# Tai-Wang/Depth-from-Motion

Hardware: NVIDIA H100
Metric: frames/sec (higher is better)
Workload: dtype f32 (bf16x2 split operands, fp32 accumulate)

## Files before the change

depth_from_motion_b200/csrc/conv_tc.cuh:

```cuda
#pragma once
#include <cuda.h>
#include <cuda_bf16.h>

#include <algorithm>
#include <cstdlib>
#include <type_traits>
#include <vector>

#include "common.cuh"
#include "simt_kernels.cuh"
#include "wgmma.cuh"

namespace dfm {

inline uint16_t bf16_rn_bits(float f) {
  uint32_t u;
  memcpy(&u, &f, 4);
  if ((u & 0x7F800000u) == 0x7F800000u) return (uint16_t)(u >> 16);
  u += 0x7FFFu + ((u >> 16) & 1u);
  return (uint16_t)(u >> 16);
}
inline float bf16_bits_to_float(uint16_t b) {
  uint32_t u = (uint32_t)b << 16;
  float f;
  memcpy(&f, &u, 4);
  return f;
}

inline int tc_sm_count() {
  int& cached = per_device<int, 1>();
  if (!cached) cudaDeviceGetAttribute(&cached, cudaDevAttrMultiProcessorCount, cur_device());
  return cached;
}

enum { TC_S1 = 0, TC_S2 = 1, TC_T = 2 };
constexpr int TC_BX = 8, TC_BY = 16;
constexpr int TC_MMA_THREADS = 256;
constexpr int TC_LOAD_THREADS = 256;
constexpr int TC_THREADS = TC_MMA_THREADS + TC_LOAD_THREADS;
constexpr int TC_MAXOPS = 9, TC_MAXBLK = 48;
constexpr int TC_ZERO_TAP = 255;

template <int MODE>
struct TcMode;
template <>
struct TcMode<TC_S1> {
  static constexpr int PXB = 10, PYB = 18, PITCH = 10, ROWS = 186, CG = 32, NSTAGE = 4;
  static constexpr int SLOT_BLOCKS = 1;
  __host__ __device__ static int zo_of(int zi, int dz) { return zi + dz; }
  __host__ __device__ static int zi_first(int zo) { return zo - 1; }
  __host__ __device__ static int zi_last(int zo) { return zo + 1; }
  __host__ __device__ static int ptype(int) { return 0; }
};
template <>
struct TcMode<TC_S2> {
  static constexpr int PXB = 17, PYB = 33, PITCH = 9, ROWS = 620, CG = 16, NSTAGE = 3;
  static constexpr int SLOT_BLOCKS = 1;
  __host__ __device__ static int zo_of(int zi, int dz) { return (zi >> 1) + dz; }
  __host__ __device__ static int zi_first(int zo) { return 2 * zo - 1; }
  __host__ __device__ static int zi_last(int zo) { return 2 * zo + 1; }
  __host__ __device__ static int ptype(int zi) { return zi & 1; }
};
template <>
struct TcMode<TC_T> {
  static constexpr int PXB = 9, PYB = 17, PITCH = 9, ROWS = 154, CG = 32, NSTAGE = 4;
  static constexpr int SLOT_BLOCKS = 4;
  __host__ __device__ static int zo_of(int zi, int dz) { return 2 * zi + dz; }
  __host__ __device__ static int zi_first(int zo) { return zo >> 1; }
  __host__ __device__ static int zi_last(int zo) { return (zo + 1) >> 1; }
  __host__ __device__ static int ptype(int) { return 0; }
};

inline int tc_mode_of(const ConvGeom& g) {
  if (g.transposed) return TC_T;
  if (g.sd == 1 && g.sh == 1 && g.sw == 1 && g.pd == 1 && g.ph == 1 && g.pw == 1) return TC_S1;
  if (g.sd == 2 && g.sh == 2 && g.sw == 2 && g.pd == 1 && g.ph == 1 && g.pw == 1 &&
      g.Di % 2 == 0 && g.Hi % 2 == 0 && g.Wi % 2 == 0)
    return TC_S2;
  return -1;
}
inline bool tc_supported(int Cin, int Cout, int ) {
  if (Cin != 32 && Cin != 64) return false;
  const int ncta = 1024 / Cin;
  return Cout % ncta == 0 && Cout <= 64;
}
inline bool tc_geom_supported(const ConvGeom& g) { return tc_mode_of(g) >= 0; }

struct TcOp {
  uint32_t a_off;
  uint32_t b_off;
  uint32_t b_lbo;
  uint16_t blk0, blk1;
  uint32_t nruns;
  uint32_t runs[3];
};
struct TcBlk {
  int8_t dz;
  uint8_t colblk;
  uint8_t tap;
  uint8_t pad;
};
struct TcProgram {
  int nops;
  uint32_t need;
  TcOp ops[TC_MAXOPS];
  TcBlk blks[TC_MAXBLK];
};

template <int MODE>
inline void tc_build_program(int ptype, int Cin, int ncta, uint32_t* w_cursor, TcProgram* pr) {
  using M = TcMode<MODE>;
  pr->nops = 0;
  pr->need = 0;
  int nb = 0;
  auto add_op = [&](int a_rows, std::vector<TcBlk> blks) {
    TcOp& op = pr->ops[pr->nops++];
    op.a_off = (uint32_t)a_rows * 16;
    op.b_off = *w_cursor;
    op.b_lbo = (uint32_t)blks.size() * ncta * 16;
    op.blk0 = (uint16_t)nb;
    for (TcBlk b : blks) pr->blks[nb++] = b;
    op.blk1 = (uint16_t)nb;
    *w_cursor += (uint32_t)(Cin / 8) * op.b_lbo;
    op.nruns = 0;
    size_t i = 0;
    while (i < blks.size()) {
      size_t e = i + 1;
      auto lin = [&](const TcBlk& b) { return (b.dz + 1) * M::SLOT_BLOCKS + b.colblk; };
      while (e < blks.size() && lin(blks[e]) == lin(blks[i]) + (int)(e - i)) ++e;
      const int nblk = (int)(e - i);
      op.runs[op.nruns++] = (uint32_t)nblk | ((uint32_t)i << 4) | ((uint32_t)lin(blks[i]) << 10);
      for (size_t k = i; k < e; ++k) pr->need |= 1u << (blks[k].dz + 1);
      i = e;
    }
  };
  if (MODE == TC_S1) {
    for (int t = 0; t < 9; ++t) {
      const int dy = t / 3, dx = t % 3;
      add_op(dy * M::PITCH + dx, {TcBlk{-1, 0, (uint8_t)(18 + t), 0}, TcBlk{0, 0, (uint8_t)(9 + t), 0},
                                  TcBlk{1, 0, (uint8_t)t, 0}});
    }
  } else if (MODE == TC_S2) {
    for (int t = 0; t < 9; ++t) {
      const int dy = t / 3, dx = t % 3;
      const int a_rows = (((dx & 1) * 2 + (dy & 1)) * 17 + (dy >> 1)) * M::PITCH + (dx >> 1);
      if (ptype == 0)
        add_op(a_rows, {TcBlk{0, 0, (uint8_t)(9 + t), 0}});
      else
        add_op(a_rows, {TcBlk{0, 0, (uint8_t)(18 + t), 0}, TcBlk{1, 0, (uint8_t)t, 0}});
    }
  } else {
    const int cls_px[4] = {0, 1, 1, 0}, cls_py[4] = {0, 0, 1, 1};
    for (int sh = 0; sh < 4; ++sh) {
      const int sx = sh & 1, sy = sh >> 1;
      std::vector<TcBlk> blks;
      for (int dz = -1; dz <= 1; ++dz) {
        const int kz = dz + 1;
        for (int c = 0; c < 4; ++c) {
          const int px = cls_px[c], py = cls_py[c];
          int kx = -1, ky = -1;
          if (px == 0) { if (!sx) kx = 1; } else kx = sx ? 0 : 2;
          if (py == 0) { if (!sy) ky = 1; } else ky = sy ? 0 : 2;
          const bool real = kx >= 0 && ky >= 0;
          blks.push_back(TcBlk{(int8_t)dz, (uint8_t)c,
                               (uint8_t)(real ? kz * 9 + ky * 3 + kx : TC_ZERO_TAP), 0});
        }
      }
      if (sh == 3) {
        std::vector<TcBlk> real;
        for (const TcBlk& b : blks)
          if (b.tap != TC_ZERO_TAP) real.push_back(b);
        blks = real;
      } else {
        while (!blks.empty() && blks.front().tap == TC_ZERO_TAP) blks.erase(blks.begin());
        while (!blks.empty() && blks.back().tap == TC_ZERO_TAP) blks.pop_back();
      }
      add_op(sy * M::PITCH + sx, blks);
    }
  }
}

struct TcWeights {
  uint8_t* dev = nullptr;
  int Cin = 0, Cout = 0, ncta = 0, nsplit = 0, mode = -1, kslice = 0;
  uint32_t image_bytes = 0, hi_bytes = 0;
  TcProgram prog[2];

  bool ready() const { return dev != nullptr; }
  void release() {
    if (dev) cudaFree(dev);
    dev = nullptr;
  }
  template <int MODE>
  bool build_mode(const float* packed, int cin, int cout, std::string* err, bool ks = false) {
    release();
    mode = MODE;
    Cin = cin;
    Cout = cout;
    kslice = ks ? 1 : 0;
    const int cin_img = ks ? 16 : cin;
    ncta = ks ? cout : 1024 / cin;
    nsplit = ks ? cin / 16 : cout / ncta;
    uint32_t cursor = 0;
    const int ntypes = MODE == TC_S2 ? 2 : 1;
    for (int t = 0; t < ntypes; ++t) tc_build_program<MODE>(t, cin_img, ncta, &cursor, &prog[t]);
    hi_bytes = cursor;
    image_bytes = 2 * hi_bytes;
    std::vector<uint16_t> img((size_t)nsplit * image_bytes / 2);
    const int kch = cin_img / 8;
    for (int s = 0; s < nsplit; ++s)
      for (int t = 0; t < ntypes; ++t)
        for (int o = 0; o < prog[t].nops; ++o) {
          const TcOp& op = prog[t].ops[o];
          const int nblk = op.blk1 - op.blk0;
          for (int kc = 0; kc < kch; ++kc)
            for (int b = 0; b < nblk; ++b)
              for (int j = 0; j < ncta; ++j)
                for (int e = 0; e < 8; ++e) {
                  const int tap = prog[t].blks[op.blk0 + b].tap;
                  if (tap == TC_ZERO_TAP) continue;
                  const int ci = kc * 8 + e + (ks ? s * 16 : 0), co = ks ? j : s * ncta + j;
                  const float w = packed[((size_t)tap * cin + ci) * cout + co];
                  const uint16_t hi = bf16_rn_bits(w);
                  const uint16_t lo = bf16_rn_bits(w - bf16_bits_to_float(hi));
                  const size_t off = (size_t)s * image_bytes / 2 + op.b_off / 2 +
                                     ((size_t)kc * nblk * ncta + (size_t)b * ncta + j) * 8 + e;
                  img[off] = hi;
                  img[off + hi_bytes / 2] = lo;
                }
        }
    if (cudaMalloc(&dev, img.size() * 2) != cudaSuccess ||
        cudaMemcpy(dev, img.data(), img.size() * 2, cudaMemcpyHostToDevice) != cudaSuccess) {
      if (err) *err = "TcWeights: device upload failed";
      release();
      return false;
    }
    return true;
  }
  bool build(const float* packed, int cin, int cout, int m, std::string* err) {
    static const bool no_ks1 = getenv("DFM_NO_KSLICE") != nullptr;
    static const bool ks1 = getenv("DFM_KSLICE_S1") != nullptr;
    if (m == TC_S1) return build_mode<TC_S1>(packed, cin, cout, err,
                                             cin == 64 && cout == 64 && !no_ks1 && ks1);
    if (m == TC_S2) {
      static const bool no_ks = getenv("DFM_NO_KSLICE") != nullptr;
      return build_mode<TC_S2>(packed, cin, cout, err, cout == 64 && !no_ks);
    }
    return build_mode<TC_T>(packed, cin, cout, err);
  }
};

__device__ __forceinline__ uint32_t smem_u32(const void* p) {
  return static_cast<uint32_t>(__cvta_generic_to_shared(p));
}
__device__ __forceinline__ void mbar_init(uint32_t bar, uint32_t count) {
  asm volatile("mbarrier.init.shared::cta.b64 [%0], %1;" ::"r"(bar), "r"(count));
}
__device__ __forceinline__ void mbar_arrive(uint32_t bar) {
  asm volatile("mbarrier.arrive.shared::cta.b64 _, [%0];" ::"r"(bar) : "memory");
}
__device__ __forceinline__ void mbar_wait(uint32_t bar, uint32_t parity, int* err) {
  for (int it = 0; it < (1 << 26); ++it) {
    uint32_t ok;
    asm volatile(
        "{\n\t.reg .pred q;\n\t"
        "mbarrier.try_wait.parity.shared::cta.b64 q, [%1], %2;\n\t"
        "selp.u32 %0, 1, 0, q;\n\t}\n"
        : "=r"(ok)
        : "r"(bar), "r"(parity)
        : "memory");
    if (ok) return;
  }
  *reinterpret_cast<volatile int*>(err) = 1;
  __threadfence_system();
}
__device__ __forceinline__ void mbar_wait_timed(uint32_t bar, uint32_t parity, int* err,
                                                unsigned long long& acc, bool timed) {
  if (!timed) {
    mbar_wait(bar, parity, err);
    return;
  }
  const long long t0 = clock64();
  mbar_wait(bar, parity, err);
  acc += (unsigned long long)(clock64() - t0);
}
__device__ __forceinline__ bool elect_one() {
  uint32_t pred;
  asm volatile(
      "{\n\t.reg .pred p;\n\telect.sync _|p, 0xffffffff;\n\tselp.u32 %0, 1, 0, p;\n\t}\n"
      : "=r"(pred));
  return pred != 0;
}
__device__ __forceinline__ void desc_add(uint64_t& d, uint32_t inc16) {
  asm("{\n\t.reg .b32 lo, hi;\n\tmov.b64 {lo, hi}, %0;\n\tadd.u32 lo, lo, %1;\n\t"
      "mov.b64 %0, {lo, hi};\n\t}\n"
      : "+l"(d)
      : "r"(inc16));
}
__device__ __forceinline__ uint64_t pack64(uint32_t lo, uint32_t hi) {
  return ((uint64_t)hi << 32) | lo;
}
__device__ __forceinline__ void split_store(const float v[8], uint8_t* hi_dst, uint8_t* lo_dst) {
  uint32_t h[4], l[4];
#pragma unroll
  for (int i = 0; i < 4; ++i) {
    const __nv_bfloat162 hh = __floats2bfloat162_rn(v[2 * i], v[2 * i + 1]);
    const float2 hf = __bfloat1622float2(hh);
    const __nv_bfloat162 ll = __floats2bfloat162_rn(v[2 * i] - hf.x, v[2 * i + 1] - hf.y);
    h[i] = *reinterpret_cast<const uint32_t*>(&hh);
    l[i] = *reinterpret_cast<const uint32_t*>(&ll);
  }
  *reinterpret_cast<uint4*>(hi_dst) = make_uint4(h[0], h[1], h[2], h[3]);
  *reinterpret_cast<uint4*>(lo_dst) = make_uint4(l[0], l[1], l[2], l[3]);
}

#ifndef DFM_LD_VARIANT
#define DFM_LD_VARIANT 0
#endif
__device__ __forceinline__ float4 ld_act(const float4* p) {
#if DFM_LD_VARIANT == 1
  return __ldcg(p);
#elif DFM_LD_VARIANT == 2
  float4 v;
  asm volatile("ld.global.nc.L1::no_allocate.L2::256B.v4.f32 {%0,%1,%2,%3}, [%4];"
               : "=f"(v.x), "=f"(v.y), "=f"(v.z), "=f"(v.w) : "l"(p));
  return v;
#elif DFM_LD_VARIANT == 3
  return __ldcs(p);
#elif DFM_LD_VARIANT == 4
  float4 v;
  asm volatile("ld.global.nc.L1::no_allocate.v4.f32 {%0,%1,%2,%3}, [%4];"
               : "=f"(v.x), "=f"(v.y), "=f"(v.z), "=f"(v.w) : "l"(p));
  return v;
#else
  return __ldg(p);
#endif
}

template <int NT>
struct SrcLoader8 {
  static constexpr bool kTma = false;
  Src s;
  int C, H, W;
  static constexpr int BATCH = 6 / NT;
  struct Raw {
    float4 a[NT][2];
  };
  __device__ __forceinline__ void issue(int z, int y, int x, int c0, Raw& r) const {
    const long long inpl = ((long long)y * W + x) * C + c0, plane = (long long)H * W * C;
#pragma unroll
    for (int t = 0; t < NT; ++t) {
      const float* px = s.t[t].x + term_plane(s.t[t], z) * plane + inpl;
      r.a[t][0] = ld_act(reinterpret_cast<const float4*>(px));
      r.a[t][1] = ld_act(reinterpret_cast<const float4*>(px) + 1);
    }
  }
  __device__ __forceinline__ void finish(const Raw& r, int c0, float v[8]) const {
#pragma unroll
    for (int i = 0; i < 8; ++i) v[i] = 0.f;
#pragma unroll
    for (int t = 0; t < NT; ++t) {
      {
        float u[8] = {r.a[t][0].x, r.a[t][0].y, r.a[t][0].z, r.a[t][0].w,
                      r.a[t][1].x, r.a[t][1].y, r.a[t][1].z, r.a[t][1].w};
        if (s.t[t].scale) {
          const float4 s0 = __ldg(reinterpret_cast<const float4*>(s.t[t].scale + c0));
          const float4 s1 = __ldg(reinterpret_cast<const float4*>(s.t[t].scale + c0) + 1);
          const float4 h0 = __ldg(reinterpret_cast<const float4*>(s.t[t].shift + c0));
          const float4 h1 = __ldg(reinterpret_cast<const float4*>(s.t[t].shift + c0) + 1);
          const float sc[8] = {s0.x, s0.y, s0.z, s0.w, s1.x, s1.y, s1.z, s1.w};
          const float sh[8] = {h0.x, h0.y, h0.z, h0.w, h1.x, h1.y, h1.z, h1.w};
#pragma unroll
          for (int i = 0; i < 8; ++i) u[i] = fmaf(u[i], sc[i], sh[i]);
        }
        if (s.t[t].relu) {
#pragma unroll
          for (int i = 0; i < 8; ++i) u[i] = fmaxf(u[i], 0.f);
        }
#pragma unroll
        for (int i = 0; i < 8; ++i) v[i] += u[i];
      }
    }
    if (s.outer_relu) {
#pragma unroll
      for (int i = 0; i < 8; ++i) v[i] = fmaxf(v[i], 0.f);
    }
  }
};

struct WarpLoader8 {
  static constexpr bool kTma = false;
  WarpLoader w;
  static constexpr int BATCH = 1;
  struct Raw {
    float4 t[4][2];
    float wt[4];
  };
  __device__ __forceinline__ void issue(int z, int y, int x, int c0, Raw& r) const {
    c0 += w.first;
    if (c0 < w.C) {
      const float* p = w.cur + ((long long)(y * w.g.step) * w.g.Wf + x * w.g.step) * w.C + c0;
      r.t[0][0] = __ldg(reinterpret_cast<const float4*>(p));
      r.t[0][1] = __ldg(reinterpret_cast<const float4*>(p) + 1);
      r.wt[0] = 1.f;
      r.wt[1] = r.wt[2] = r.wt[3] = 0.f;
      return;
    }
    c0 -= w.C;
    float fx, fy;
    warp_coord(w.g, x, y, __ldg(w.depths + z), fx, fy);
    const Taps t = bilinear_taps(fx, fy, w.g.Hf, w.g.Wf);
#pragma unroll
    for (int k = 0; k < 4; ++k) {
      r.wt[k] = t.w[k];
      if (t.w[k] != 0.f) {
        const float* p = w.prev + (long long)t.off[k] * w.C + c0;
        r.t[k][0] = __ldg(reinterpret_cast<const float4*>(p));
        r.t[k][1] = __ldg(reinterpret_cast<const float4*>(p) + 1);
      }
    }
  }
  __device__ __forceinline__ void finish(const Raw& r, int, float v[8]) const {
#pragma unroll
    for (int i = 0; i < 8; ++i) v[i] = 0.f;
#pragma unroll
    for (int k = 0; k < 4; ++k) {
      if (r.wt[k] != 0.f) {
        v[0] = fmaf(r.wt[k], r.t[k][0].x, v[0]); v[1] = fmaf(r.wt[k], r.t[k][0].y, v[1]);
        v[2] = fmaf(r.wt[k], r.t[k][0].z, v[2]); v[3] = fmaf(r.wt[k], r.t[k][0].w, v[3]);
        v[4] = fmaf(r.wt[k], r.t[k][1].x, v[4]); v[5] = fmaf(r.wt[k], r.t[k][1].y, v[5]);
        v[6] = fmaf(r.wt[k], r.t[k][1].z, v[6]); v[7] = fmaf(r.wt[k], r.t[k][1].w, v[7]);
      }
    }
  }
};

struct TmaLoader8 {
  static constexpr bool kTma = true;
  static constexpr int BATCH = 1;
  CUtensorMap map;
  int nch_total;
  struct Raw {};
  __device__ __forceinline__ void issue(int, int, int, int, Raw&) const {}
  __device__ __forceinline__ void finish(const Raw&, int, float v[8]) const {
#pragma unroll
    for (int i = 0; i < 8; ++i) v[i] = 0.f;
  }
};
constexpr int TMA_S2_CLS = 17 * 9;
constexpr int TMA_S2_CLSR = (2 * TMA_S2_CLS + 7) / 8 * 8;

__device__ __forceinline__ void tma_load_4d(uint32_t dst, const CUtensorMap* map, int c1, int c2,
                                            int c3, uint32_t bar) {
  asm volatile(
      "cp.async.bulk.tensor.4d.shared::cluster.global.tile.mbarrier::complete_tx::bytes "
      "[%0], [%1, {%2, %3, %4, %5}], [%6];" ::"r"(dst),
      "l"(map), "r"(0), "r"(c1), "r"(c2), "r"(c3), "r"(bar)
      : "memory");
}

constexpr int PS_XRUN = 64, PS_WARPS = 4, PS_SEG = 33;
inline size_t presplit_smem_bytes(int C) { return (size_t)PS_WARPS * 4 * (C / 8) * PS_SEG * 16; }
template <int NT>
__global__ void __launch_bounds__(32 * PS_WARPS)
presplit_kernel(const SrcLoader8<NT> ld, int Z, uint4* __restrict__ out) {
  extern __shared__ uint4 ps_sm[];
  const int nch = ld.C >> 3, W = ld.W, H = ld.H, W2 = W >> 1, H2 = H >> 1;
  const int warp = threadIdx.x >> 5, lane = threadIdx.x & 31;
  uint4* sm = ps_sm + (size_t)warp * 4 * nch * PS_SEG;
  const int runs_per_row = (W + PS_XRUN - 1) / PS_XRUN;
  const long long nruns = (long long)Z * H * runs_per_row;
  for (long long r = (long long)blockIdx.x * PS_WARPS + warp; r < nruns;
       r += (long long)gridDim.x * PS_WARPS) {
    const int run = (int)(r % runs_per_row);
    const long long zy = r / runs_per_row;
    const int y = (int)(zy % H), z = (int)(zy / H);
    const int xb = run * PS_XRUN;
#pragma unroll 4
    for (int i = lane; i < PS_XRUN * nch; i += 32) {
      const int xl = i / nch, chunk = i - xl * nch, x = xb + xl;
      if (x < W) {
        typename SrcLoader8<NT>::Raw raw;
        ld.issue(z, y, x, chunk * 8, raw);
        float val[8];
        ld.finish(raw, chunk * 8, val);
        uint4* hi = sm + ((xl & 1) * nch + chunk) * PS_SEG + (xl >> 1);
        split_store(val, reinterpret_cast<uint8_t*>(hi),
                    reinterpret_cast<uint8_t*>(hi + 2 * nch * PS_SEG));
      }
    }
    __syncwarp();
    const int py = y & 1, y2 = y >> 1, x2 = (xb >> 1) + lane;
    for (int seg = 0; seg < 4 * nch; ++seg) {
      const int chunk = seg % nch, px = (seg / nch) & 1, hl = seg / (2 * nch);
      if (2 * x2 + px < W)
        out[((((long long)(z * 2 + hl) * 4 + py * 2 + px) * nch + chunk) * H2 + y2) * W2 + x2] =
            sm[seg * PS_SEG + lane];
    }
    __syncwarp();
  }
}
inline bool presplit_launch(const Src& s, int C, int Z, int H, int W, uint4* out, cudaStream_t st) {
  if ((H | W) & 1) return false;
  const size_t smem = presplit_smem_bytes(C);
  const long long nruns = (long long)Z * H * ((W + PS_XRUN - 1) / PS_XRUN);
  const int blocks = (int)std::min<long long>((nruns + PS_WARPS - 1) / PS_WARPS, 12LL * tc_sm_count());
  auto go = [&](auto kern, auto ld) {
    if (cudaFuncSetAttribute(kern, cudaFuncAttributeMaxDynamicSharedMemorySize, (int)smem) !=
        cudaSuccess)
      return false;
    kern<<<blocks, 32 * PS_WARPS, smem, st>>>(ld, Z, out);
    return cudaGetLastError() == cudaSuccess;
  };
  if (s.n == 1) return go(presplit_kernel<1>, SrcLoader8<1>{s, C, H, W});
  if (s.n == 2) return go(presplit_kernel<2>, SrcLoader8<2>{s, C, H, W});
  return go(presplit_kernel<3>, SrcLoader8<3>{s, C, H, W});
}

inline bool make_presplit_map_s2(CUtensorMap* map, const void* base, int W, int H,
                                 long long slabs, std::string* err) {
  typedef CUresult (*EncodeFn)(CUtensorMap*, CUtensorMapDataType, cuuint32_t, void*,
                               const cuuint64_t*, const cuuint64_t*, const cuuint32_t*,
                               const cuuint32_t*, CUtensorMapInterleave, CUtensorMapSwizzle,
                               CUtensorMapL2promotion, CUtensorMapFloatOOBfill);
  static EncodeFn encode = nullptr;
  if (!encode) {
    void* fn = nullptr;
    cudaDriverEntryPointQueryResult qres;
    if (cudaGetDriverEntryPoint("cuTensorMapEncodeTiled", &fn, cudaEnableDefault, &qres) !=
            cudaSuccess || !fn || qres != cudaDriverEntryPointSuccess) {
      if (err) *err = "cuTensorMapEncodeTiled is not available from this driver";
      return false;
    }
    encode = (EncodeFn)fn;
  }
  const int W2 = W / 2, H2 = H / 2;
  const cuuint64_t dims[4] = {8, (cuuint64_t)W2, (cuuint64_t)H2, (cuuint64_t)slabs};
  const cuuint64_t strides[3] = {16, (cuuint64_t)W2 * 16, (cuuint64_t)H2 * W2 * 16};
  const cuuint32_t box[4] = {8, 9, 17, 2};
  const cuuint32_t estr[4] = {1, 1, 1, 1};
  const CUresult r = encode(map, CU_TENSOR_MAP_DATA_TYPE_UINT16, 4, const_cast<void*>(base), dims,
                            strides, box, estr, CU_TENSOR_MAP_INTERLEAVE_NONE,
                            CU_TENSOR_MAP_SWIZZLE_NONE, CU_TENSOR_MAP_L2_PROMOTION_L2_128B,
                            CU_TENSOR_MAP_FLOAT_OOB_FILL_NONE);
  if (r != CUDA_SUCCESS) {
    if (err) *err = "cuTensorMapEncodeTiled failed with code " + std::to_string((int)r);
    return false;
  }
  return true;
}

struct TcParams {
  const uint8_t* wimg;
  float* out;
  double* stats;
  int Di, Hi, Wi;
  int Do, Ho, Wo, Cout;
  int Mx, My;
  int tiles_x, tiles_y, nsplit;
  int z_unit;
  uint32_t w_bytes, w_hi_bytes;
  int* err;
  unsigned long long* role_cycles;
  const float* addend;
  int zw_lo, zw_hi;
  float zw;
  long long slice_stride;
  int store1;
  int dbg;
};

struct TcItem {
  int x0, y0, split, z_lo, z_hi;
};
struct TcWalk {
  long long cur, end;
  int split;
};
__device__ __forceinline__ TcWalk tc_walk_begin(const TcParams& p) {
  TcWalk w;
  const int per_split = gridDim.x / p.nsplit;
  w.split = blockIdx.x % p.nsplit;
  const int r = blockIdx.x / p.nsplit;
  const long long units_col = p.Do / p.z_unit;
  const long long total = (long long)p.tiles_x * p.tiles_y * units_col;
  w.cur = total * r / per_split;
  w.end = total * (r + 1) / per_split;
  return w;
}
__device__ __forceinline__ bool tc_walk_next(const TcParams& p, TcWalk& w, TcItem& it) {
  if (w.cur >= w.end) return false;
  const long long units_col = p.Do / p.z_unit;
  const int col = (int)(w.cur / units_col);
  const long long u0 = w.cur % units_col;
  const long long u1 = min(units_col, u0 + (w.end - w.cur));
  it.split = w.split;
  it.x0 = (col % p.tiles_x) * TC_BX;
  it.y0 = (col / p.tiles_x) * TC_BY;
  it.z_lo = (int)u0 * p.z_unit;
  it.z_hi = (int)u1 * p.z_unit;
  w.cur += u1 - u0;
  return true;
}

template <int MODE>
struct TcWin;
template <>
struct TcWin<TC_S1> {
  static constexpr int NPL = 3;
  __device__ static int base(int zi) { return zi - 1; }
};
template <>
struct TcWin<TC_S2> {
  static constexpr int NPL = 2;
  __device__ static int base(int zi) { return zi >> 1; }
};
template <>
struct TcWin<TC_T> {
  static constexpr int NPL = 3;
  __device__ static int base(int zi) { return 2 * zi - 1; }
};

template <int MODE, int CIN, int NCTA, class Loader>
__global__ void __launch_bounds__(TC_THREADS, 1) conv_tc_kernel(const __grid_constant__ TcParams p,
                                                                 const __grid_constant__ Loader ld) {
  using M = TcMode<MODE>;
  using Win = TcWin<MODE>;
  constexpr bool TMA = Loader::kTma;
  static_assert(!TMA || MODE == TC_S2, "the TMA loader serves the stride-2 brick only");
  constexpr int CG = M::CG < CIN ? M::CG : CIN;
  constexpr int NCH = CG / 8;
  constexpr int NCG = CIN / CG;
  static_assert(!TMA || NCH == 2, "TMA stride-2 stages hold two 8-channel chunks");
  constexpr uint32_t S2_CLS16 = TMA ? TMA_S2_CLSR : TMA_S2_CLS;
  constexpr uint32_t A_LBO = TMA ? TMA_S2_CLS * 16 : M::ROWS * 16;
  constexpr uint32_t A_SBO = M::PITCH * 16;
  constexpr uint32_t A_HL = TMA ? 4 * TMA_S2_CLSR * 16 : NCH * M::ROWS * 16;
  constexpr uint32_t STAGE_BYTES = 2 * A_HL;
  constexpr uint32_t B_SBO = 128;
  constexpr bool KSLICE = CIN == 16;
  constexpr int NPOS = M::PXB * M::PYB;
  constexpr int LGROUPS = 2;
  constexpr int LG_THREADS = TC_LOAD_THREADS / LGROUPS;
  constexpr int NITEM = (NPOS * NCH + LG_THREADS - 1) / LG_THREADS;
  constexpr int PCOLS = M::SLOT_BLOCKS * NCTA;
  constexpr int NACC = Win::NPL * PCOLS / 2;

  extern __shared__ __align__(1024) uint8_t smem[];
  uint8_t* w_s = smem;
  uint8_t* a_s = smem + p.w_bytes;
  uint64_t* bars = reinterpret_cast<uint64_t*>(a_s + M::NSTAGE * STAGE_BYTES);

  const int tid = threadIdx.x, lane = tid & 31;
  const int warp = __shfl_sync(0xffffffffu, tid >> 5, 0);
  const uint32_t bar0 = smem_u32(bars);
  auto full_a = [&](int s) { return bar0 + 8u * s; };
  auto empty_a = [&](int s) { return bar0 + 8u * (M::NSTAGE + s); };
  const uint32_t w_bar = bar0 + 8u * (2 * M::NSTAGE);
  constexpr int LOAD_WARP0 = TC_MMA_THREADS / 32;

  if (tid == 0) {
    for (int s = 0; s < M::NSTAGE; ++s) {
      mbar_init(full_a(s), TMA ? 1 : LG_THREADS / 32);
      mbar_init(empty_a(s), TC_MMA_THREADS / 32);
    }
    mbar_init(w_bar, 1);
    asm volatile("fence.mbarrier_init.release.cluster;" ::: "memory");
    const int split = blockIdx.x % p.nsplit;
    const uint8_t* src = p.wimg + (size_t)split * p.w_bytes;
    asm volatile("mbarrier.arrive.expect_tx.shared::cta.b64 _, [%0], %1;" ::"r"(w_bar),
                 "r"(p.w_bytes)
                 : "memory");
    constexpr uint32_t CHUNK = 32768;
    for (uint32_t off = 0; off < p.w_bytes; off += CHUNK) {
      const uint32_t n = min(CHUNK, p.w_bytes - off);
      asm volatile(
          "cp.async.bulk.shared::cluster.global.mbarrier::complete_tx::bytes [%0], [%1], %2, [%3];"
          ::"r"(smem_u32(w_s + off)), "l"(src + off), "r"(n), "r"(w_bar)
          : "memory");
    }
  }
  __syncthreads();

  if constexpr (TMA) {
    if (warp == LOAD_WARP0 && lane == 0) {
      constexpr uint32_t STAGE_TX = 8u * 2u * TMA_S2_CLS * 16u;
      uint32_t stage_ctr = 0;
      TcWalk walk = tc_walk_begin(p);
      TcItem it;
      while (tc_walk_next(p, walk, it)) {
        const int zi0 = max(M::zi_first(it.z_lo), 0);
        const int zi1 = min(M::zi_last(it.z_hi - 1), p.Di - 1);
        const int chunk0 = CIN == 16 ? it.split * 2 : 0;
        for (int zi = zi0; zi <= zi1; ++zi) {
#pragma unroll 1
          for (int cg = 0; cg < NCG; ++cg, ++stage_ctr) {
            const int s = stage_ctr % M::NSTAGE;
            mbar_wait(empty_a(s), ((stage_ctr / M::NSTAGE) & 1) ^ 1, p.err);
            asm volatile("mbarrier.arrive.expect_tx.shared::cta.b64 _, [%0], %1;" ::"r"(full_a(s)),
                         "r"(STAGE_TX)
                         : "memory");
            const uint32_t st_addr = smem_u32(a_s + s * STAGE_BYTES);
#pragma unroll
            for (int hl = 0; hl < 2; ++hl) {
#pragma unroll
              for (int cls = 0; cls < 4; ++cls) {
                const int bxp = cls >> 1, byp = cls & 1;
                const int cls_in = (1 - byp) * 2 + (1 - bxp);
                const int slab = ((zi * 2 + hl) * 4 + cls_in) * ld.nch_total + chunk0 + cg * NCH;
                tma_load_4d(st_addr + hl * A_HL + cls * (TMA_S2_CLSR * 16), &ld.map,
                            it.x0 - 1 + bxp, it.y0 - 1 + byp, slab, full_a(s));
              }
            }
          }
        }
      }
    }
  }
  if (TMA && warp >= LOAD_WARP0) {
  } else if (warp >= LOAD_WARP0) {
    const int lw = warp - LOAD_WARP0;
    const int lgrp = lw & (LGROUPS - 1);
    const int lt = (lw / LGROUPS) * 32 + lane;
    const int chunk = lt % NCH;
    uint32_t stage_ctr = 0;
    const bool timed = p.role_cycles != nullptr && lw == 0 && lane == 0;
    unsigned long long t_wait_e = 0;
    const long long t_begin = clock64();
    TcWalk walk = tc_walk_begin(p);
    TcItem it;
    while (tc_walk_next(p, walk, it)) {
      int soff[NITEM], gx[NITEM], gy[NITEM];
      bool inb[NITEM], live[NITEM];
#pragma unroll
      for (int k = 0; k < NITEM; ++k) {
        const int i = lt + k * LG_THREADS;
        live[k] = i < NPOS * NCH;
        const int pos = i / NCH;
        const int bx = pos % M::PXB, by = pos / M::PXB;
        int row;
        if (MODE == TC_S1) {
          gx[k] = it.x0 - 1 + bx;
          gy[k] = it.y0 - 1 + by;
          row = by * M::PITCH + bx;
        } else if (MODE == TC_S2) {
          gx[k] = 2 * it.x0 - 1 + bx;
          gy[k] = 2 * it.y0 - 1 + by;
          row = (((bx & 1) * 2 + (by & 1)) * 17 + (by >> 1)) * M::PITCH + (bx >> 1);
        } else {
          gx[k] = it.x0 + bx;
          gy[k] = it.y0 + by;
          row = by * M::PITCH + bx;
        }
        inb[k] = live[k] && gx[k] >= 0 && gx[k] < p.Wi && gy[k] >= 0 && gy[k] < p.Hi;
        soff[k] = (chunk * M::ROWS + row) * 16;
      }
      const int zi0 = max(M::zi_first(it.z_lo), 0);
      const int zi1 = min(M::zi_last(it.z_hi - 1), p.Di - 1);
      for (int zi = zi0; zi <= zi1; ++zi) {
#pragma unroll 1
        for (int cg = 0; cg < NCG; ++cg, ++stage_ctr) {
          if ((int)(stage_ctr & (LGROUPS - 1)) != lgrp) continue;
          const int s = stage_ctr % M::NSTAGE;
          mbar_wait_timed(empty_a(s), ((stage_ctr / M::NSTAGE) & 1) ^ 1, p.err, t_wait_e, timed);
          uint8_t* st = a_s + s * STAGE_BYTES;
          const int c0 = cg * CG + chunk * 8 + (KSLICE ? it.split * CIN : 0);
          constexpr int LB = Loader::BATCH < NITEM ? Loader::BATCH : NITEM;
          if (!(p.dbg & 1))
#pragma unroll
          for (int k0 = 0; k0 < NITEM; k0 += LB) {
            typename Loader::Raw raw[LB];
#pragma unroll
            for (int b = 0; b < LB; ++b)
              if (k0 + b < NITEM && inb[k0 + b] && !(p.dbg & 16))
                ld.issue(zi, gy[k0 + b], gx[k0 + b], c0, raw[b]);
#pragma unroll
            for (int b = 0; b < LB; ++b) {
              if (k0 + b < NITEM && live[k0 + b]) {
                float v[8];
                if (inb[k0 + b]) {
                  ld.finish(raw[b], c0, v);
                } else {
#pragma unroll
                  for (int i = 0; i < 8; ++i) v[i] = 0.f;
                }
                if (!(p.dbg & 32)) split_store(v, st + soff[k0 + b], st + A_HL + soff[k0 + b]);
                else if (v[0] + v[1] + v[2] + v[3] + v[4] + v[5] + v[6] + v[7] == 1.2345f) st[0] = 1;
              }
            }
          }
          if (!(p.dbg & 8)) asm volatile("fence.proxy.async.shared::cta;" ::: "memory");
          __syncwarp();
          if (lane == 0) mbar_arrive(full_a(s));
        }
      }
    }
    if (timed) {
      unsigned long long* rc = p.role_cycles + (size_t)blockIdx.x * 8;
      rc[3] = (unsigned long long)(clock64() - t_begin);
      rc[4] = t_wait_e;
    }
  } else {
    const int wg = warp >> 2, wq = warp & 3;
    const bool timed = p.role_cycles != nullptr && tid == 0;
    unsigned long long t_wait_a = 0;
    const long long t_begin = clock64();
    mbar_wait(w_bar, 0u, p.err);
    const uint32_t w_base = smem_u32(w_s), a_base = smem_u32(a_s);
    constexpr uint32_t A_LBO16 = A_LBO >> 4, A_HL16 = A_HL >> 4;
    const uint32_t a_desc_hi = A_SBO >> 4;
    const uint32_t b_desc_hi = B_SBO >> 4;
    const uint32_t w_hi16 = p.w_hi_bytes >> 4;
    const uint32_t a_wg16 = (uint32_t)wg * 8u * (A_SBO >> 4);

    float acc[NACC];
#pragma unroll
    for (int i = 0; i < NACC; ++i) acc[i] = 0.f;
    constexpr int NST = KSLICE ? 1 : NCTA / 4;
    float ssum[NST], ssq[NST];
#pragma unroll
    for (int i = 0; i < NST; ++i) ssum[i] = ssq[i] = 0.f;

    const int xr = lane >> 2, cq = lane & 3;
    auto flush_stats = [&](int split) {
      if (KSLICE || !p.stats) return;
#pragma unroll
      for (int k = 0; k < NST; ++k) {
        double a = ssum[k], b = ssq[k];
#pragma unroll
        for (int o = 4; o < 32; o <<= 1) {
          a += __shfl_xor_sync(0xffffffffu, a, o);
          b += __shfl_xor_sync(0xffffffffu, b, o);
        }
        if (lane < 4) {
          const int ch = split * NCTA + 8 * (k >> 1) + 2 * lane + (k & 1);
          atomicAdd(p.stats + 2 * ch, a);
          atomicAdd(p.stats + 2 * ch + 1, b);
        }
        ssum[k] = ssq[k] = 0.f;
      }
    };
    auto emit = [&](const TcItem& it, auto jc, int zo) {
      constexpr int J = decltype(jc)::value;
      if (zo < it.z_lo || zo >= it.z_hi) return;
#pragma unroll
      for (int cb = 0; cb < M::SLOT_BLOCKS; ++cb) {
        const float* r = acc + (J * PCOLS + cb * NCTA) / 2;
#pragma unroll
        for (int rr = 0; rr < 2; ++rr) {
          const int mx = it.x0 + xr, my = it.y0 + 8 * wg + 2 * wq + rr;
          if (mx >= p.Mx || my >= p.My) continue;
          int xo = mx, yo = my;
          if (MODE == TC_T) {
            xo = 2 * mx + ((cb == 1 || cb == 2) ? 1 : 0);
            yo = 2 * my + (cb >= 2 ? 1 : 0);
          }
          const long long vox = ((long long)zo * p.Ho + yo) * p.Wo + xo;
          if (p.store1) {
            if (cq == 0) p.out[vox] = r[2 * rr];
            continue;
          }
          const int ch_base = (KSLICE ? 0 : it.split * NCTA) + 2 * cq;
          const float wz = (zo >= p.zw_lo && zo < p.zw_hi) ? p.zw : 1.f;
#pragma unroll
          for (int j = 0; j < NCTA / 8; ++j) {
            float v0 = r[4 * j + 2 * rr], v1 = r[4 * j + 2 * rr + 1];
            const int ch = ch_base + 8 * j;
            if (p.addend) {
              const int cls = zo == 0 ? 0 : (zo == p.Do - 1 ? 2 : 1);
              const float2 a2 = __ldg(reinterpret_cast<const float2*>(
                  p.addend + (((long long)cls * p.Ho + yo) * p.Wo + xo) * p.Cout + ch));
              v0 += a2.x;
              v1 += a2.y;
            }
            *reinterpret_cast<float2*>(p.out + (KSLICE ? it.split * p.slice_stride : 0) +
                                       vox * p.Cout + ch) = make_float2(v0, v1);
            if constexpr (!KSLICE) {
              if (p.stats) {
                ssum[2 * j] = fmaf(wz, v0, ssum[2 * j]);
                ssq[2 * j] = fmaf(wz * v0, v0, ssq[2 * j]);
                ssum[2 * j + 1] = fmaf(wz, v1, ssum[2 * j + 1]);
                ssq[2 * j + 1] = fmaf(wz * v1, v1, ssq[2 * j + 1]);
              }
            }
          }
        }
      }
    };
    auto shift = [&](auto shc) {
      constexpr int SH = decltype(shc)::value * PCOLS / 2;
#pragma unroll
      for (int i = 0; i < NACC; ++i) acc[i] = i + SH < NACC ? acc[i + SH] : 0.f;
    };

    uint32_t stage_ctr = 0;
    TcWalk walk = tc_walk_begin(p);
    TcItem it;
    while (tc_walk_next(p, walk, it)) {
      const int zi0 = max(M::zi_first(it.z_lo), 0);
      const int zi1 = min(M::zi_last(it.z_hi - 1), p.Di - 1);
      for (int zi = zi0; zi <= zi1; ++zi) {
#pragma unroll 1
        for (int cg = 0; cg < NCG; ++cg, ++stage_ctr) {
          const int s = stage_ctr % M::NSTAGE;
          mbar_wait_timed(full_a(s), (stage_ctr / M::NSTAGE) & 1, p.err, t_wait_a, timed);
          __syncwarp();
          const uint32_t a_lo_stage =
              ((((a_base + s * STAGE_BYTES) >> 4) & 0x3FFF) + a_wg16) | (A_LBO16 << 16);
          wgmma_fence();
          if constexpr (MODE == TC_S1) {
            constexpr uint32_t B_LBO16 = 3 * NCTA;
            constexpr uint32_t TAP16 = (CIN / 8) * B_LBO16;
            constexpr int NKS = CG / 16;
            const uint32_t b_lo0 = ((w_base >> 4) & 0x3FFF) + (uint32_t)(cg * NCH) * B_LBO16 +
                                   (B_LBO16 << 16);
            uint64_t da[NKS][2], db[NKS][2];
#pragma unroll
            for (int ks = 0; ks < NKS; ++ks) {
              da[ks][0] = pack64(a_lo_stage + 2 * ks * A_LBO16, a_desc_hi);
              da[ks][1] = pack64(a_lo_stage + 2 * ks * A_LBO16 + A_HL16, a_desc_hi);
              const uint32_t bl = b_lo0 + 2 * ks * B_LBO16;
              db[ks][0] = pack64(bl, b_desc_hi);
              db[ks][1] = pack64(bl + w_hi16, b_desc_hi);
            }
#pragma unroll 1
            for (int tap = 0; tap < 9; ++tap) {
#pragma unroll
              for (int ks = 0; ks < NKS; ++ks) {
                wgmma_bf16<3 * NCTA>(acc, da[ks][0], db[ks][0]);
                wgmma_bf16<3 * NCTA>(acc, da[ks][1], db[ks][0]);
                wgmma_bf16<3 * NCTA>(acc, da[ks][0], db[ks][1]);
              }
              const uint32_t ainc = (tap == 2 || tap == 5) ? (uint32_t)(M::PITCH - 2) : 1u;
#pragma unroll
              for (int ks = 0; ks < NKS; ++ks) {
                desc_add(da[ks][0], ainc);
                desc_add(da[ks][1], ainc);
                desc_add(db[ks][0], TAP16);
                desc_add(db[ks][1], TAP16);
              }
            }
          }
          if constexpr (MODE == TC_S2) {
            constexpr uint32_t KCH16 = CIN / 8;
            const uint32_t odd = (uint32_t)zi & 1u;
            auto run = [&](auto nbc) {
              constexpr uint32_t NB = decltype(nbc)::value;
              constexpr uint32_t b_lbo16 = NB * NCTA;
              constexpr uint32_t tap16 = KCH16 * b_lbo16;
              const uint32_t b_lo0 = ((w_base >> 4) & 0x3FFF) + (NB == 2 ? 9u * KCH16 * NCTA : 0u) +
                                     (uint32_t)(cg * NCH) * b_lbo16 + (b_lbo16 << 16);
              uint64_t dbh = pack64(b_lo0, b_desc_hi);
              uint64_t dbl = pack64(b_lo0 + w_hi16, b_desc_hi);
#pragma unroll
              for (int tap = 0; tap < 9; ++tap) {
                const int dy = tap / 3, dx = tap % 3;
                const uint32_t a16 = (uint32_t)(((dx & 1) * 2 + (dy & 1)) * S2_CLS16 +
                                                (dy >> 1) * M::PITCH + (dx >> 1));
                const uint64_t dah = pack64(a_lo_stage + a16, a_desc_hi);
                const uint64_t dal = pack64(a_lo_stage + a16 + A_HL16, a_desc_hi);
                wgmma_bf16<NB * NCTA>(acc, dah, dbh);
                wgmma_bf16<NB * NCTA>(acc, dal, dbh);
                wgmma_bf16<NB * NCTA>(acc, dah, dbl);
                desc_add(dbh, tap16);
                desc_add(dbl, tap16);
              }
            };
            if (odd) run(std::integral_constant<uint32_t, 2>());
            else run(std::integral_constant<uint32_t, 1>());
          }
          if constexpr (MODE == TC_T) {
            constexpr uint32_t KCH16 = CIN / 8;
            constexpr uint32_t NB[4] = {12u, 10u, 10u, 3u};
            constexpr uint32_t LIN0[4] = {0u, 1u, 2u, 2u};
            uint32_t b_img16 = (w_base >> 4) & 0x3FFF;
#pragma unroll
            for (int sh = 0; sh < 4; ++sh) {
              const uint32_t b_lbo16 = NB[sh] * NCTA;
              const uint32_t a16 = (uint32_t)((sh >> 1) * M::PITCH + (sh & 1));
#pragma unroll
              for (int ks = 0; ks < CG / 16; ++ks) {
                const uint32_t alo = a_lo_stage + a16 + 2 * ks * A_LBO16;
                const uint64_t dah = pack64(alo, a_desc_hi);
                const uint64_t dal = pack64(alo + A_HL16, a_desc_hi);
                const uint32_t blo = b_img16 + (uint32_t)(cg * NCH + 2 * ks) * b_lbo16 +
                                     (b_lbo16 << 16);
                auto mma3 = [&](float* d, uint32_t bl, auto nc) {
                  constexpr int N = decltype(nc)::value;
                  const uint64_t dbh = pack64(bl, b_desc_hi);
                  const uint64_t dbl = pack64(bl + w_hi16, b_desc_hi);
                  wgmma_bf16<N>(d, dah, dbh);
                  wgmma_bf16<N>(d, dal, dbh);
                  wgmma_bf16<N>(d, dah, dbl);
                };
                if (sh == 0) {
                  mma3(acc, blo, std::integral_constant<int, 12 * NCTA>());
                } else if (sh == 1) {
                  mma3(acc + NCTA / 2, blo, std::integral_constant<int, 10 * NCTA>());
                } else if (sh == 2) {
                  mma3(acc + NCTA, blo, std::integral_constant<int, 10 * NCTA>());
                } else {
#pragma unroll
                  for (uint32_t k = 0; k < 3; ++k)
                    mma3(acc + (LIN0[3] + k * 4) * (NCTA / 2), blo + k * NCTA,
                         std::integral_constant<int, NCTA>());
                }
              }
              b_img16 += KCH16 * b_lbo16;
            }
          }
          wgmma_commit();
          wgmma_wait<0>();
          __syncwarp();
          if (lane == 0) mbar_arrive(empty_a(s));
        }
        if constexpr (MODE == TC_S1) {
          emit(it, std::integral_constant<int, 0>(), zi - 1);
          shift(std::integral_constant<int, 1>());
        } else if constexpr (MODE == TC_S2) {
          if (zi & 1) {
            emit(it, std::integral_constant<int, 0>(), zi >> 1);
            shift(std::integral_constant<int, 1>());
          }
        } else {
          emit(it, std::integral_constant<int, 0>(), 2 * zi - 1);
          emit(it, std::integral_constant<int, 1>(), 2 * zi);
          shift(std::integral_constant<int, 2>());
        }
      }
      const int zb = Win::base(zi1 + 1);
      emit(it, std::integral_constant<int, 0>(), zb);
      emit(it, std::integral_constant<int, 1>(), zb + 1);
      if constexpr (Win::NPL > 2) emit(it, std::integral_constant<int, 2>(), zb + 2);
#pragma unroll
      for (int i = 0; i < NACC; ++i) acc[i] = 0.f;
      flush_stats(it.split);
    }
    if (timed) {
      unsigned long long* rc = p.role_cycles + (size_t)blockIdx.x * 8;
      rc[0] = (unsigned long long)(clock64() - t_begin);
      rc[1] = t_wait_a;
    }
  }
}

struct TcErrFlag {
  int* host = nullptr;
  int* dev = nullptr;
  int* get() {
    if (!host) {
      if (cudaHostAlloc(&host, sizeof(int), cudaHostAllocMapped | cudaHostAllocPortable) !=
          cudaSuccess) {
        host = nullptr;
        cudaGetLastError();
        return nullptr;
      }
      *host = 0;
      cudaHostGetDevicePointer(&dev, host, 0);
    }
    return dev;
  }
};
inline TcErrFlag& tc_err_flag() {
  static TcErrFlag f;
  return f;
}
inline int tc_consume_error() {
  TcErrFlag& f = tc_err_flag();
  if (!f.host) return 0;
  const int h = *reinterpret_cast<volatile int*>(f.host);
  if (h) *reinterpret_cast<volatile int*>(f.host) = 0;
  return h;
}

__global__ void __launch_bounds__(256)
kslice_reduce_kernel(const float* __restrict__ part, int nsl, long long V, long long HW,
                     float* __restrict__ out, double* __restrict__ stats, int zw_lo, int zw_hi,
                     float zw) {
  __shared__ double sh[2][16][64];
  const int q = threadIdx.x & 15, r = threadIdx.x >> 4;
  double s[4] = {0, 0, 0, 0}, ss[4] = {0, 0, 0, 0};
  const long long w0 = (long long)zw_lo * HW, w1 = (long long)zw_hi * HW;
  for (long long v = (long long)blockIdx.x * 16 + r; v < V; v += (long long)gridDim.x * 16) {
    float4 a = __ldg(reinterpret_cast<const float4*>(part + v * 64) + q);
    for (int k = 1; k < nsl; ++k) {
      const float4 b = __ldg(reinterpret_cast<const float4*>(part + ((long long)k * V + v) * 64) + q);
      a.x += b.x; a.y += b.y; a.z += b.z; a.w += b.w;
    }
    reinterpret_cast<float4*>(out + v * 64)[q] = a;
    if (stats) {
      const double wgt = (v >= w0 && v < w1) ? (double)zw : 1.0;
      s[0] += wgt * a.x; ss[0] += wgt * (double)a.x * a.x;
      s[1] += wgt * a.y; ss[1] += wgt * (double)a.y * a.y;
      s[2] += wgt * a.z; ss[2] += wgt * (double)a.z * a.z;
      s[3] += wgt * a.w; ss[3] += wgt * (double)a.w * a.w;
    }
  }
  if (!stats) return;
#pragma unroll
  for (int i = 0; i < 4; ++i) {
    sh[0][r][4 * q + i] = s[i];
    sh[1][r][4 * q + i] = ss[i];
  }
  __syncthreads();
  if (threadIdx.x < 128) {
    const int c = threadIdx.x & 63, which = threadIdx.x >> 6;
    double t = 0.0;
    for (int k = 0; k < 16; ++k) t += sh[which][k][c];
    atomicAdd(stats + 2 * c + which, t);
  }
}
struct TcScratch {
  float* p = nullptr;
  size_t n = 0;
  float* get(size_t count) {
    if (n >= count) return p;
    if (p) cudaFree(p);
    p = nullptr;
    n = 0;
    if (cudaMalloc(&p, count * sizeof(float)) != cudaSuccess) return nullptr;
    n = count;
    return p;
  }
};
inline TcScratch& tc_kslice_scratch() { return per_device<TcScratch>(); }

struct TcOpts {
  int store1 = 0;
  const float* addend = nullptr;
  int zw_lo = 0, zw_hi = 0;
  float zw = 1.f;
  long long slice_stride = 0;
};
template <int MODE, int CIN, int NCTA, class Loader>
bool tc_launch(const Loader& ld, const TcWeights& w, float* out, double* stats,
               const ConvGeom& g, cudaStream_t st, std::string* err, TcOpts opt = TcOpts()) {
  using M = TcMode<MODE>;
  constexpr int CG = M::CG < CIN ? M::CG : CIN;
  constexpr size_t STAGE_BYTES = Loader::kTma ? (size_t)2 * 4 * TMA_S2_CLSR * 16
                                              : (size_t)2 * (CG / 8) * M::ROWS * 16;
  const size_t smem = w.image_bytes + M::NSTAGE * STAGE_BYTES + (2 * M::NSTAGE + 1) * 8;
  auto kern = conv_tc_kernel<MODE, CIN, NCTA, Loader>;
  struct AttrTag { size_t v = 0; };
  static AttrTag attr_dev[kMaxDevices];
  size_t& attr_smem = attr_dev[cur_device()].v;
  if (smem > attr_smem) {
    if (smem > 232448 ||
        cudaFuncSetAttribute(kern, cudaFuncAttributeMaxDynamicSharedMemorySize, (int)smem) !=
            cudaSuccess) {
      if (err) *err = "conv_tc: cannot reserve " + std::to_string(smem) + " B of shared memory";
      return false;
    }
    attr_smem = smem;
  }
  const int sms = tc_sm_count();
  TcParams p{};
  p.wimg = w.dev;
  p.out = out;
  p.stats = stats;
  p.store1 = opt.store1;
  p.slice_stride = opt.slice_stride;
  p.addend = opt.addend;
  p.zw_lo = opt.zw_lo;
  p.zw_hi = opt.zw_hi;
  p.zw = opt.zw;
  p.Di = g.Di; p.Hi = g.Hi; p.Wi = g.Wi;
  p.Do = g.Do; p.Ho = g.Ho; p.Wo = g.Wo;
  p.Cout = g.Cout;
  p.Mx = MODE == TC_T ? g.Wi : g.Wo;
  p.My = MODE == TC_T ? g.Hi : g.Ho;
  p.tiles_x = (p.Mx + TC_BX - 1) / TC_BX;
  p.tiles_y = (p.My + TC_BY - 1) / TC_BY;
  p.nsplit = w.nsplit;
  p.w_bytes = w.image_bytes;
  p.w_hi_bytes = w.hi_bytes;
  p.z_unit = MODE == TC_T ? 2 : 1;
  const long long cols = (long long)p.tiles_x * p.tiles_y;
  const long long units = cols * (g.Do / p.z_unit);
  int per_split = std::max(1, sms / p.nsplit);
  per_split = (int)std::min<long long>(per_split, units);
  const int grid = per_split * p.nsplit;
  p.err = tc_err_flag().get();
  static const bool role_dbg = getenv("DFM_TC_ROLE_CYCLES") != nullptr;
  static const int dbg_flags = getenv("DFM_TC_DEBUG") ? atoi(getenv("DFM_TC_DEBUG")) : 0;
  p.dbg = dbg_flags;
  static unsigned long long* role_buf = nullptr;
  if (role_dbg) {
    if (!role_buf) cudaMalloc(&role_buf, 1024 * 8 * sizeof(unsigned long long));
    cudaMemsetAsync(role_buf, 0, 1024 * 8 * sizeof(unsigned long long), st);
    p.role_cycles = role_buf;
  }
  kern<<<grid, TC_THREADS, smem, st>>>(p, ld);
  if (role_dbg) {
    cudaStreamSynchronize(st);
    std::vector<unsigned long long> h((size_t)grid * 8);
    cudaMemcpy(h.data(), role_buf, h.size() * 8, cudaMemcpyDeviceToHost);
    double a[8] = {0};
    for (int b = 0; b < grid; ++b)
      for (int k = 0; k < 8; ++k) a[k] += (double)h[(size_t)b * 8 + k] / grid;
    fprintf(stderr,
            "[tc mode=%d cin=%d ncta=%d grid=%d cols=%lld Do=%d] mma+epilogue: total %.0f "
            "wait_full_a %.0f | load: total %.0f wait_empty_a %.0f\n",
            MODE, CIN, NCTA, grid, cols, g.Do, a[0], a[1], a[3], a[4]);
  }
  const cudaError_t e = cudaGetLastError();
  if (e != cudaSuccess) {
    if (err) *err = std::string("conv_tc launch: ") + cudaGetErrorString(e);
    return false;
  }
  return true;
}

template <class Loader>
bool tc_dispatch(const Loader& ld, const TcWeights& w, float* out, double* stats,
                 const ConvGeom& g, cudaStream_t st, std::string* err, TcOpts opt = TcOpts()) {
  const int mode = tc_mode_of(g);
  if (mode != w.mode) {
    if (err) *err = "conv_tc: weight image was built for a different conv mode";
    return false;
  }
  if (w.kslice) {
    if ((mode != TC_S2 && mode != TC_S1) || g.Cout != 64 || opt.addend || opt.store1) {
      if (err) *err = "conv_tc: K-slice weights are for plain convs with 64 outputs";
      return false;
    }
    const long long V = (long long)g.Do * g.Ho * g.Wo;
    float* part = tc_kslice_scratch().get((size_t)w.nsplit * V * 64);
    if (!part) {
      if (err) *err = "conv_tc: cannot allocate the K-slice scratch";
      return false;
    }
    TcOpts o2 = opt;
    o2.slice_stride = V * 64;
    bool launched = false;
    if constexpr (Loader::kTma) {
      if (mode == TC_S2) launched = tc_launch<TC_S2, 16, 64, Loader>(ld, w, part, nullptr, g, st, err, o2);
      else if (err) *err = "conv_tc: the TMA loader serves stride-2 convs only";
    } else {
      launched = mode == TC_S2
                     ? tc_launch<TC_S2, 16, 64, Loader>(ld, w, part, nullptr, g, st, err, o2)
                     : tc_launch<TC_S1, 16, 64, Loader>(ld, w, part, nullptr, g, st, err, o2);
    }
    if (!launched) return false;
    const int blocks = (int)std::min<long long>(8LL * tc_sm_count(), (V + 15) / 16);
    kslice_reduce_kernel<<<blocks, 256, 0, st>>>(part, w.nsplit, V, (long long)g.Ho * g.Wo, out,
                                                 stats, opt.zw_lo, opt.zw_hi, opt.zw);
    if (cudaGetLastError() != cudaSuccess) {
      if (err) *err = "conv_tc: kslice_reduce_kernel launch failed";
      return false;
    }
    return true;
  }
  if constexpr (Loader::kTma) {
    if (err) *err = "conv_tc: the TMA loader serves the K-slice stride-2 convs only";
    return false;
  } else {
#define TC_CASE(MD, CI, NC) \
  if (mode == MD && g.Cin == CI) \
    return tc_launch<MD, CI, NC, Loader>(ld, w, out, stats, g, st, err, opt)
  TC_CASE(TC_S1, 32, 32);
  TC_CASE(TC_S1, 64, 16);
  TC_CASE(TC_S2, 32, 32);
  TC_CASE(TC_S2, 64, 16);
  TC_CASE(TC_T, 64, 16);
#undef TC_CASE
  if (err) *err = "conv_tc: unsupported (mode, Cin)";
  return false;
  }
}

inline bool tc_conv_src(const Src& s, const TcWeights& w, float* out, double* stats,
                        const ConvGeom& g, cudaStream_t st, std::string* err,
                        TcOpts opt = TcOpts()) {
  if (s.n == 1) {
    SrcLoader8<1> ld{s, g.Cin, g.Hi, g.Wi};
    return tc_dispatch(ld, w, out, stats, g, st, err, opt);
  }
  if (s.n == 2) {
    SrcLoader8<2> ld{s, g.Cin, g.Hi, g.Wi};
    return tc_dispatch(ld, w, out, stats, g, st, err, opt);
  }
  SrcLoader8<3> ld{s, g.Cin, g.Hi, g.Wi};
  return tc_dispatch(ld, w, out, stats, g, st, err, opt);
}
inline bool tc_conv_presplit(const uint4* ps, int channels, const TcWeights& w, float* out,
                             double* stats, const ConvGeom& g, cudaStream_t st, std::string* err,
                             TcOpts opt = TcOpts()) {
  if (tc_mode_of(g) != TC_S2 || !w.kslice || channels != g.Cin) {
    if (err) *err = "conv_tc: the TMA loader serves the K-slice stride-2 convs only";
    return false;
  }
  TmaLoader8 ld;
  ld.nch_total = channels / 8;
  if (!make_presplit_map_s2(&ld.map, ps, g.Wi, g.Hi, (long long)g.Di * 2 * 4 * ld.nch_total, err))
    return false;
  return tc_dispatch(ld, w, out, stats, g, st, err, opt);
}
inline bool tc_conv_warp(const WarpLoader& wl, const TcWeights& w, float* out, double* stats,
                         const ConvGeom& g, cudaStream_t st, std::string* err,
                         TcOpts opt = TcOpts()) {
  if (tc_mode_of(g) != TC_S1) {
    if (err) *err = "conv_tc: the warp loader feeds stride-1 convs only";
    return false;
  }
  WarpLoader8 ld{wl};
  if (g.Cin == 32)
    return tc_launch<TC_S1, 32, 32, WarpLoader8>(ld, w, out, stats, g, st, err, opt);
  if (g.Cin == 64)
    return tc_launch<TC_S1, 64, 16, WarpLoader8>(ld, w, out, stats, g, st, err, opt);
  if (err) *err = "conv_tc: unsupported Cin";
  return false;
}

}
```

Baseline: 84.22.

## Reorder transposed-conv accumulators class-major and shrink TMA loader to one warp

The transposed-conv tap program now orders weight blocks class-major (per output parity class, then dz), and the accumulator layout is changed to match. This removes zero-padded weight blocks, so the shifted-parity wgmma calls use narrower N (6*NCTA instead of 10*NCTA) and the last shift becomes one MMA instead of three. The run-encoding metadata goes away. Separately, when the loader uses TMA, the kernel launches with a single 32-thread load warp instead of 256 load threads, which reduces the block size and register pressure.

```diff
diff --git a/depth_from_motion_b200/csrc/conv_tc.cuh b/depth_from_motion_b200/csrc/conv_tc.cuh
--- a/depth_from_motion_b200/csrc/conv_tc.cuh
+++ b/depth_from_motion_b200/csrc/conv_tc.cuh
@@ -36,10 +36,7 @@
 enum { TC_S1 = 0, TC_S2 = 1, TC_T = 2 };
 constexpr int TC_BX = 8, TC_BY = 16;
 constexpr int TC_MMA_THREADS = 256;
-constexpr int TC_LOAD_THREADS = 256;
-constexpr int TC_THREADS = TC_MMA_THREADS + TC_LOAD_THREADS;
 constexpr int TC_MAXOPS = 9, TC_MAXBLK = 48;
-constexpr int TC_ZERO_TAP = 255;
 
 template <int MODE>
 struct TcMode;
@@ -71,6 +68,15 @@
   __host__ __device__ static int ptype(int) { return 0; }
 };
 
+template <bool TMA>
+__host__ __device__ constexpr int tc_load_threads() {
+  return TMA ? 32 : 256;
+}
+template <bool TMA>
+__host__ __device__ constexpr int tc_threads() {
+  return TC_MMA_THREADS + tc_load_threads<TMA>();
+}
+
 inline int tc_mode_of(const ConvGeom& g) {
   if (g.transposed) return TC_T;
   if (g.sd == 1 && g.sh == 1 && g.sw == 1 && g.pd == 1 && g.ph == 1 && g.pw == 1) return TC_S1;
@@ -91,8 +97,6 @@
   uint32_t b_off;
   uint32_t b_lbo;
   uint16_t blk0, blk1;
-  uint32_t nruns;
-  uint32_t runs[3];
 };
 struct TcBlk {
   int8_t dz;
@@ -119,20 +123,12 @@
     op.b_off = *w_cursor;
     op.b_lbo = (uint32_t)blks.size() * ncta * 16;
     op.blk0 = (uint16_t)nb;
-    for (TcBlk b : blks) pr->blks[nb++] = b;
+    for (TcBlk b : blks) {
+      pr->blks[nb++] = b;
+      pr->need |= 1u << (b.dz + 1);
+    }
     op.blk1 = (uint16_t)nb;
     *w_cursor += (uint32_t)(Cin / 8) * op.b_lbo;
-    op.nruns = 0;
-    size_t i = 0;
-    while (i < blks.size()) {
-      size_t e = i + 1;
-      auto lin = [&](const TcBlk& b) { return (b.dz + 1) * M::SLOT_BLOCKS + b.colblk; };
-      while (e < blks.size() && lin(blks[e]) == lin(blks[i]) + (int)(e - i)) ++e;
-      const int nblk = (int)(e - i);
-      op.runs[op.nruns++] = (uint32_t)nblk | ((uint32_t)i << 4) | ((uint32_t)lin(blks[i]) << 10);
-      for (size_t k = i; k < e; ++k) pr->need |= 1u << (blks[k].dz + 1);
-      i = e;
-    }
   };
   if (MODE == TC_S1) {
     for (int t = 0; t < 9; ++t) {
@@ -154,26 +150,14 @@
     for (int sh = 0; sh < 4; ++sh) {
       const int sx = sh & 1, sy = sh >> 1;
       std::vector<TcBlk> blks;
-      for (int dz = -1; dz <= 1; ++dz) {
-        const int kz = dz + 1;
-        for (int c = 0; c < 4; ++c) {
-          const int px = cls_px[c], py = cls_py[c];
-          int kx = -1, ky = -1;
-          if (px == 0) { if (!sx) kx = 1; } else kx = sx ? 0 : 2;
-          if (py == 0) { if (!sy) ky = 1; } else ky = sy ? 0 : 2;
-          const bool real = kx >= 0 && ky >= 0;
-          blks.push_back(TcBlk{(int8_t)dz, (uint8_t)c,
-                               (uint8_t)(real ? kz * 9 + ky * 3 + kx : TC_ZERO_TAP), 0});
-        }
-      }
-      if (sh == 3) {
-        std::vector<TcBlk> real;
-        for (const TcBlk& b : blks)
-          if (b.tap != TC_ZERO_TAP) real.push_back(b);
-        blks = real;
-      } else {
-        while (!blks.empty() && blks.front().tap == TC_ZERO_TAP) blks.erase(blks.begin());
-        while (!blks.empty() && blks.back().tap == TC_ZERO_TAP) blks.pop_back();
+      for (int c = 0; c < 4; ++c) {
+        const int px = cls_px[c], py = cls_py[c];
+        int kx = -1, ky = -1;
+        if (px == 0) { if (!sx) kx = 1; } else kx = sx ? 0 : 2;
+        if (py == 0) { if (!sy) ky = 1; } else ky = sy ? 0 : 2;
+        if (kx < 0 || ky < 0) continue;
+        for (int dz = -1; dz <= 1; ++dz)
+          blks.push_back(TcBlk{(int8_t)dz, (uint8_t)c, (uint8_t)((dz + 1) * 9 + ky * 3 + kx), 0});
       }
       add_op(sy * M::PITCH + sx, blks);
     }
@@ -218,7 +202,6 @@
               for (int j = 0; j < ncta; ++j)
                 for (int e = 0; e < 8; ++e) {
                   const int tap = prog[t].blks[op.blk0 + b].tap;
-                  if (tap == TC_ZERO_TAP) continue;
                   const int ci = kc * 8 + e + (ks ? s * 16 : 0), co = ks ? j : s * ncta + j;
                   const float w = packed[((size_t)tap * cin + ci) * cout + co];
                   const uint16_t hi = bf16_rn_bits(w);
@@ -622,8 +605,8 @@
 };
 
 template <int MODE, int CIN, int NCTA, class Loader>
-__global__ void __launch_bounds__(TC_THREADS, 1) conv_tc_kernel(const __grid_constant__ TcParams p,
-                                                                 const __grid_constant__ Loader ld) {
+__global__ void __launch_bounds__((tc_threads<Loader::kTma>()), 1)
+    conv_tc_kernel(const __grid_constant__ TcParams p, const __grid_constant__ Loader ld) {
   using M = TcMode<MODE>;
   using Win = TcWin<MODE>;
   constexpr bool TMA = Loader::kTma;
@@ -641,10 +624,9 @@
   constexpr bool KSLICE = CIN == 16;
   constexpr int NPOS = M::PXB * M::PYB;
   constexpr int LGROUPS = 2;
-  constexpr int LG_THREADS = TC_LOAD_THREADS / LGROUPS;
-  constexpr int NITEM = (NPOS * NCH + LG_THREADS - 1) / LG_THREADS;
-  constexpr int PCOLS = M::SLOT_BLOCKS * NCTA;
-  constexpr int NACC = Win::NPL * PCOLS / 2;
+  constexpr int LG_THREADS = tc_load_threads<TMA>() / LGROUPS;
+  constexpr int NITEM = TMA ? 1 : (NPOS * NCH + LG_THREADS - 1) / LG_THREADS;
+  constexpr int NACC = M::SLOT_BLOCKS * Win::NPL * NCTA / 2;
 
   extern __shared__ __align__(1024) uint8_t smem[];
   uint8_t* w_s = smem;
@@ -682,8 +664,8 @@
   }
   __syncthreads();
 
-  if constexpr (TMA) {
-    if (warp == LOAD_WARP0 && lane == 0) {
+  if (TMA && warp >= LOAD_WARP0) {
+    if constexpr (TMA) if (lane == 0) {
       constexpr uint32_t STAGE_TX = 8u * 2u * TMA_S2_CLS * 16u;
       uint32_t stage_ctr = 0;
       TcWalk walk = tc_walk_begin(p);
@@ -716,8 +698,6 @@
         }
       }
     }
-  }
-  if (TMA && warp >= LOAD_WARP0) {
   } else if (warp >= LOAD_WARP0) {
     const int lw = warp - LOAD_WARP0;
     const int lgrp = lw & (LGROUPS - 1);
@@ -845,7 +825,7 @@
       if (zo < it.z_lo || zo >= it.z_hi) return;
 #pragma unroll
       for (int cb = 0; cb < M::SLOT_BLOCKS; ++cb) {
-        const float* r = acc + (J * PCOLS + cb * NCTA) / 2;
+        const float* r = acc + (cb * Win::NPL + J) * NCTA / 2;
 #pragma unroll
         for (int rr = 0; rr < 2; ++rr) {
           const int mx = it.x0 + xr, my = it.y0 + 8 * wg + 2 * wq + rr;
@@ -888,9 +868,11 @@
       }
     };
     auto shift = [&](auto shc) {
-      constexpr int SH = decltype(shc)::value * PCOLS / 2;
-#pragma unroll
-      for (int i = 0; i < NACC; ++i) acc[i] = i + SH < NACC ? acc[i + SH] : 0.f;
+      constexpr int SH = decltype(shc)::value * NCTA / 2, PL = Win::NPL * NCTA / 2;
+#pragma unroll
+      for (int cb = 0; cb < M::SLOT_BLOCKS; ++cb)
+#pragma unroll
+        for (int i = 0; i < PL; ++i) acc[cb * PL + i] = i + SH < PL ? acc[cb * PL + i + SH] : 0.f;
     };
 
     uint32_t stage_ctr = 0;
@@ -971,8 +953,8 @@
           }
           if constexpr (MODE == TC_T) {
             constexpr uint32_t KCH16 = CIN / 8;
-            constexpr uint32_t NB[4] = {12u, 10u, 10u, 3u};
-            constexpr uint32_t LIN0[4] = {0u, 1u, 2u, 2u};
+            constexpr uint32_t NB[4] = {12u, 6u, 6u, 3u};
+            constexpr uint32_t CLS0[4] = {0u, 1u, 2u, 2u};
             uint32_t b_img16 = (w_base >> 4) & 0x3FFF;
 #pragma unroll
             for (int sh = 0; sh < 4; ++sh) {
@@ -993,18 +975,10 @@
                   wgmma_bf16<N>(d, dal, dbh);
                   wgmma_bf16<N>(d, dah, dbl);
                 };
-                if (sh == 0) {
-                  mma3(acc, blo, std::integral_constant<int, 12 * NCTA>());
-                } else if (sh == 1) {
-                  mma3(acc + NCTA / 2, blo, std::integral_constant<int, 10 * NCTA>());
-                } else if (sh == 2) {
-                  mma3(acc + NCTA, blo, std::integral_constant<int, 10 * NCTA>());
-                } else {
-#pragma unroll
-                  for (uint32_t k = 0; k < 3; ++k)
-                    mma3(acc + (LIN0[3] + k * 4) * (NCTA / 2), blo + k * NCTA,
-                         std::integral_constant<int, NCTA>());
-                }
+                float* d = acc + CLS0[sh] * Win::NPL * (NCTA / 2);
+                if (sh == 0) mma3(d, blo, std::integral_constant<int, 12 * NCTA>());
+                else if (sh < 3) mma3(d, blo, std::integral_constant<int, 6 * NCTA>());
+                else mma3(d, blo, std::integral_constant<int, 3 * NCTA>());
               }
               b_img16 += KCH16 * b_lbo16;
             }
@@ -1190,7 +1164,7 @@
     cudaMemsetAsync(role_buf, 0, 1024 * 8 * sizeof(unsigned long long), st);
     p.role_cycles = role_buf;
   }
-  kern<<<grid, TC_THREADS, smem, st>>>(p, ld);
+  kern<<<grid, tc_threads<Loader::kTma>(), smem, st>>>(p, ld);
   if (role_dbg) {
     cudaStreamSynchronize(st);
     std::vector<unsigned long long> h((size_t)grid * 8);
```

After: 86.88 (median of 6 runs). 3.2% higher.
